# caskcsg/lightretriever

Hardware: AMD Instinct MI355X
Metric: docs embedded/sec (llama3.2-1b dims, seq_len=512, bf16) [+ queries/sec@top-100 over 1000000-doc index in `search`] (higher is better)
Workload: dtype bf16

## Files before the change

lightretriever_amd/csrc/lrx_search.hip:

```cpp
#include "lrx_common.h"
#include <float.h>
#include <stdlib.h>

typedef const __attribute__((address_space(1))) void* gptr_t;
typedef __attribute__((address_space(3))) void* lptr_t;

#define ROWS_F32 0
#define ROWS_F16T 1

#include "lrx_search_filter.h"

extern "C" int64_t lrx_flat_ip_score_ld(int64_t n_rows) { return lrx_cdiv(n_rows > 0 ? n_rows : 1, S_ROWS) * S_ROWS; }

#define SPLIT_MIN_QT 3
static size_t split_ws_bytes(int32_t dim) { return (size_t)(dim / 32) * 3 * 8 * 1024; }

struct FilterMode {
  int bmode = 0;
  int ss = 1;
  int unit = 1;
  int64_t nblocks = -1;
  const float* thr = nullptr;
  unsigned long long* cand = nullptr;
  unsigned int* cnt = nullptr;
  unsigned int cap = CAND_CAP_MIN;
  int* zero = nullptr;
  int nzero = 0;
  PreSplit presplit;
  bool planes_ready = false;
  bool group_max = false;
  const struct FusedArgs* fused = nullptr;
  bool range = false;
};
struct FusedArgs {
  int64_t ld_s;
  int nblk_s, nblk_ld_s, nsamp, nmain, ss, k;
  const float* bounds;
  float *thr, *eps;
  unsigned long long* cand;
  unsigned int* cnt;
  unsigned int cap;
  FusedCtl* ctl;
  int phases;
  int rs;
};

static int lrx_cu_count() {
  static const int n_cu = []() {
    int dev = 0;
    hipDeviceProp_t prop;
    return (hipGetDevice(&dev) == hipSuccess && hipGetDeviceProperties(&prop, dev) == hipSuccess && prop.multiProcessorCount > 0) ? prop.multiProcessorCount : 256;
  }();
  return n_cu;
}

static int filter_rows_per_wg(bool shadow) { return shadow ? 128 : 16 * SPF_RT * SPF_WV; }
template <int RS>
static int launch_filter_fused(const void* Xs, int64_t n_rows, int dim, const __bf16* qsplit, int nq, int qt, float* scores, float* gmax, const float* qf32,
                               const FusedArgs& fa, hipStream_t s);

static int launch_scores(const float* X, int64_t n_rows, int64_t ldx, int32_t dim, const float* q, int32_t n_queries, float* scores,
                         float* blkmax, __bf16* qsplit, void* stream, int planes = 3, const int* gate = nullptr, const void* Xs = nullptr,
                         int64_t ld = 0, const FilterMode& fm = FilterMode()) {
  LRX_CHECK_ARG(dim > 0 && dim % S_BK == 0, "flat_ip: dim=%d must be a multiple of %d", dim, S_BK);
  LRX_CHECK_ARG(ldx >= dim && ldx % 4 == 0, "flat_ip: ldx=%lld must be >= dim and a multiple of 4", (long long)ldx);
  if (n_rows <= 0 || n_queries <= 0) return LRX_OK;
  const int64_t ld_full = lrx_flat_ip_score_ld(n_rows);
  if (ld == 0) ld = ld_full;
  const int nblk_ld = (int)((ld / SP_ROWS + 3) & ~3);
  dim3 block(256);
  hipStream_t s = (hipStream_t)stream;
  const bool emit = fm.cand != nullptr;
  const bool shadow_pass = qsplit != nullptr && planes == 1 && Xs != nullptr;
  const int chunk = shadow_pass ? 256 : 128;
  LRX_CHECK_ARG(fm.bmode == 0 || (planes == 1 && qsplit != nullptr && n_queries <= chunk), "flat_ip: sampled filter launch outside the bounded search");
  for (int q0 = 0; q0 < n_queries; q0 += chunk) {
    int nq = n_queries - q0 < chunk ? n_queries - q0 : chunk;
    int qt = (nq + 15) / 16;
    const float* qp = q + (int64_t)q0 * dim;
    float* sp = scores ? scores + (int64_t)q0 * ld : nullptr;
    float* bp = blkmax ? blkmax + (int64_t)q0 * nblk_ld : nullptr;
    if (shadow_pass) {
      const int64_t nwg = fm.nblocks >= 0 ? fm.nblocks : ld_full / 128;
      if (nwg == 0) continue;
      if (fm.bmode != 2) {
        int threads = (dim / 64) * 2 * qt * 64;
        PreSplit ps = fm.presplit;
        ps.nb_xb = (threads + 255) / 256;
        hipLaunchKernelGGL(k_pack_queries_xb, dim3(ps.nb_xb + (ps.ngroups > 0 ? ps.blocks[0] + ps.blocks[1] : 0)), dim3(256), 0, s, qp, nq, dim, qt, qsplit,
                           fm.zero, fm.nzero, ps);
      }
      if (fm.fused != nullptr) {
        const int rc = fm.fused->rs == ROWS_F16T ? launch_filter_fused<ROWS_F16T>(Xs, n_rows, dim, qsplit, nq, qt, sp, bp, qp, *fm.fused, s)
                                                 : launch_filter_fused<ROWS_F32>(Xs, n_rows, dim, qsplit, nq, qt, sp, bp, qp, *fm.fused, s);
        if (rc != LRX_OK) return rc;
        continue;
      }
      constexpr int XPF = 4;
#ifndef XPF_S
#define XPF_S 4
#endif
      const int n_cu = lrx_cu_count();
      const bool persistent = emit && gate == nullptr && (dim / 64) % XPF == 0 && fm.bmode != 1 && nwg < (1ll << 31);
      const bool two_blocks = !emit && fm.bmode == 1 && nwg < (1ll << 31) && nwg > lrx_cu_count();
      const bool persistent_store = two_blocks && fm.group_max && gate == nullptr && sp != nullptr && bp != nullptr && qt <= 8 && (dim / 64) % XPF == 0 &&
                                    (nwg + 1) / 2 > 2 * (int64_t)n_cu;
#define LRX_XP(QQ, RT_)                                                                                                                     \
  {                                                                                                                                         \
    const int64_t groups = (nwg + RT_ - 1) / RT_;                                                                                           \
    if (fm.range)                                                                                                                           \
      hipLaunchKernelGGL((k_filter_xreg_emit<QQ, (QQ == 8 ? 2 : XPF), RT_, true>), dim3((unsigned)(groups < n_cu ? groups : n_cu)), dim3(576), 0, s, \
                         (const __bf16*)Xs, n_rows, dim, qsplit, nq, (int)nwg, fm.bmode, fm.ss, fm.unit, fm.thr, fm.cand, fm.cnt, fm.cap);     \
    else                                                                                                                                    \
    hipLaunchKernelGGL((k_filter_xreg_emit<QQ, (QQ == 8 ? 2 : XPF), RT_>), dim3((unsigned)(groups < n_cu ? groups : n_cu)), dim3(576), 0, s, (const __bf16*)Xs, n_rows, \
                       dim, qsplit, nq, (int)nwg, fm.bmode, fm.ss, fm.unit, fm.thr, fm.cand, fm.cnt, fm.cap);                              \
  }
#define LRX_XN(QQ, EM_)                                                                                                                     \
  hipLaunchKernelGGL((k_filter_xreg<QQ, (EM_ ? XPF : XPF_S), EM_>), dim3((unsigned)nwg), dim3(576), 0, s, (const __bf16*)Xs, n_rows, dim, qsplit, nq, sp, ld, bp, \
                     nblk_ld, gate, fm.bmode, fm.ss, fm.unit, fm.thr, fm.cand, fm.cnt, (int)nwg, fm.group_max ? 1 : 0, fm.cap);
#define LRX_XN2(QQ)                                                                              \
  hipLaunchKernelGGL((k_filter_xreg<QQ, XPF, false, 2>), dim3((unsigned)((nwg + 1) / 2)), dim3(576), 0, s, (const __bf16*)Xs, n_rows, dim, qsplit, nq, sp, ld, bp, \
                     nblk_ld, gate, fm.bmode, fm.ss, fm.unit, fm.thr, fm.cand, fm.cnt, (int)nwg, fm.group_max ? 1 : 0, fm.cap);
#define LRX_XS(QQ)                                                     \
// ... 236 lines not shown
extern "C" int32_t lrx_flat_ip_bounded_chunk_queries(int64_t n_rows, int32_t dim, int32_t n_queries, int32_t k, int32_t flags, int32_t has_shadow) {
  return chunk_queries(n_rows, dim, n_queries > 0 ? n_queries : 1, k, has_shadow && dim % 64 == 0, flags & 3);
}

static size_t chunk_plans_bytes(int64_t n_rows, int32_t dim, int32_t nq, int32_t k, int mode, bool shadow) {
  size_t need = 0;
  const int chunk = chunk_queries(n_rows, dim, nq, k, shadow, mode);
  const int sizes[2] = {nq < chunk ? nq : chunk, nq > chunk ? nq % chunk : 0};
  for (int i = 0; i < 2; ++i)
    if (sizes[i] > 0) {
      size_t t = plan_chunk(n_rows, dim, sizes[i], k, shadow, mode, 0).total;
      const size_t tf = plan_chunk(n_rows, dim, sizes[i], k, shadow, mode, 1).total;
      t = tf > t ? tf : t;
      need = t > need ? t : need;
    }
  return need;
}

extern "C" size_t lrx_flat_ip_bounded_workspace_bytes(int64_t n_rows, int32_t dim, int32_t n_queries, int32_t k, int32_t flags) {
  const int32_t nq = n_queries > 0 ? n_queries : 1;
  const size_t need = lrx_flat_ip_workspace_bytes(n_rows, dim, nq < 128 ? nq : 128, k);
  const size_t a = chunk_plans_bytes(n_rows, dim, nq, k, flags & 3, false), b = chunk_plans_bytes(n_rows, dim, nq, k, flags & 3, true);
  const size_t m = a > b ? a : b;
  return (m > need ? m : need) + 512;
}

extern "C" int lrx_flat_ip_search_bounded(const float* X, int64_t n_rows, int64_t ldx, int32_t dim, const void* X_shadow, const float* row_bounds,
                                          const float* q, int32_t n_queries, int32_t k, int64_t id_base, float* out_scores, int64_t* out_ids,
                                          void* workspace, size_t workspace_bytes, int32_t flags, void* stream) {
  return lrx_flat_ip_search_bounded_wire(X, n_rows, ldx, dim, X_shadow, row_bounds, q, n_queries, k, id_base, out_scores, out_ids, nullptr, nullptr,
                                         workspace, workspace_bytes, flags, stream);
}

template <int RS>
static int bounded_search(const float* X, int64_t n_rows, int64_t ldx, int32_t dim, const void* X_shadow, const float* row_bounds,
                          const float* q, int32_t n_queries, int32_t k, int64_t id_base, float* out_scores, int64_t* out_ids,
                          const int64_t* row_map, uint64_t* out_wire, void* workspace, size_t workspace_bytes, int32_t flags, void* stream) {
  const int mode = flags & 3;
  const bool shadow = X_shadow != nullptr && dim % 64 == 0;
  const int qt_max = ((n_queries < 128 ? n_queries : 128) + 15) / 16;
  if (RS == ROWS_F32 && ((qt_max < SPLIT_MIN_QT && !shadow) || n_rows <= REF_CAND || dim % 4 != 0)) {
    for (int q0 = 0; q0 < n_queries; q0 += 128) {
      const int nq = n_queries - q0 < 128 ? n_queries - q0 : 128;
      const int rc = lrx_flat_ip_search(X, n_rows, ldx, dim, row_bounds, q + (int64_t)q0 * dim, nq, k, id_base, out_scores + (int64_t)q0 * k,
                                        out_ids + (int64_t)q0 * k, workspace, workspace_bytes, stream);
      if (rc != LRX_OK) return rc;
    }
    return out_wire != nullptr ? lrx_pack_topk(out_scores, out_ids, row_map, id_base, (int64_t)n_queries * k, out_wire, stream) : LRX_OK;
  }
  hipStream_t s = (hipStream_t)stream;
  const int chunk = chunk_queries(n_rows, dim, n_queries, k, shadow, mode);
  const int use_fused = fused_pref_of(flags);
  for (int q0 = 0; q0 < n_queries; q0 += chunk) {
    const int nq = n_queries - q0 < chunk ? n_queries - q0 : chunk;
    const BoundedPlan p = plan_chunk(n_rows, dim, nq, k, shadow, mode, use_fused);
    LRX_CHECK_ARG(nq <= (shadow ? 256 : 128) || (p.gemm && p.emit), "flat_ip_search_bounded: a chunk of %d queries without the GEMM main pass", nq);
    if (p.total > workspace_bytes) {
      lrx_set_error("flat_ip_search_bounded: chunk of %d queries needs %zu B of workspace, %zu given", nq, p.total, workspace_bytes);
      return LRX_ERR_WORKSPACE;
    }
    const float* qc = q + (int64_t)q0 * dim;
    float* osc = out_scores + (int64_t)q0 * k;
    int64_t* oic = out_ids + (int64_t)q0 * k;
    char* ws = (char*)workspace;
    float* scores = (float*)ws;
    __bf16* qsplit = (__bf16*)(ws + p.off_qsplit);
    int* flg = (int*)(ws + p.off_ints);
    int* any_flag = flg + nq;
    unsigned int* cnt = (unsigned int*)(flg + ints_before_cnt(nq));
    int* part_cnt = (int*)(cnt + (size_t)nq * CNT_STRIDE);
    float* thr = (float*)(part_cnt + (size_t)nq * REF_SPLIT);
    float* eps = thr + nq;
    unsigned long long* parts = (unsigned long long*)(ws + p.off_parts);
    unsigned long long* cand = (unsigned long long*)(ws + p.off_cand);
    const size_t nclear = ints_before_cnt(nq) + (p.emit ? (size_t)nq * CNT_STRIDE : 0);
    const bool clear_in_pack = shadow && nclear < (1u << 30);
    if (!clear_in_pack) LRX_HIP(hipMemsetAsync(flg, 0, sizeof(int) * nclear, s));
    __bf16* qs3 = (__bf16*)(ws + p.off_qs3);
    const int64_t qs3_stride = (int64_t)(split_ws_bytes(dim) / sizeof(__bf16));
    auto presplit_of = [&](int j) {
      PreSplit ps;
      if (!shadow || RS == ROWS_F16T) return ps;
      const int n0 = j * 256, nj = nq - n0 < 256 ? nq - n0 : 256;
      ps.qs3 = qs3 + (int64_t)(2 * j) * qs3_stride;
      ps.stride = qs3_stride;
      for (int f0 = 0, g = 0; f0 < nj; f0 += 128, ++g) {
        const int nf = nj - f0 < 128 ? nj - f0 : 128, qtf = (nf + 15) / 16;
        ps.nf[g] = nf;
        ps.qt[g] = qtf;
        ps.blocks[g] = qtf >= SPLIT_MIN_QT ? ((dim / 32) * qtf * 64 + 255) / 256 : 0;
        ps.ngroups = g + 1;
      }
      if (ps.blocks[0] + ps.blocks[1] == 0) ps.ngroups = 0;
      return ps;
    };
    const PreSplit presplit = presplit_of(0);
    int rc;
    int nsplit = REF_SPLIT;
    if (p.emit) {
      float* blkmax = scores + p.ld_s * (int64_t)nq;
      FilterMode fs;
      fs.bmode = 1; fs.ss = p.ss; fs.unit = 1; fs.nblocks = p.nsamp_wg;
      fs.group_max = shadow;
      if (clear_in_pack) { fs.zero = flg; fs.nzero = (int)nclear; }
      fs.presplit = presplit;
      FusedArgs fa;
      if (p.fused && clear_in_pack) {
        fa.ld_s = p.ld_s; fa.nblk_s = (int)p.nblk_s; fa.nblk_ld_s = (int)p.nblk_ld_s; fa.nsamp = (int)p.nsamp_wg; fa.nmain = (int)p.nmain_wg; fa.ss = p.ss; fa.k = k;
        fa.bounds = row_bounds; fa.thr = thr; fa.eps = eps; fa.cand = cand; fa.cnt = cnt; fa.cap = p.cap;
        fa.ctl = (FusedCtl*)(flg + ints_before_cnt(nq) - 8);
        static const int fused_stamps = lrx_dev_knob("LRX_FUSED_PHASES", 0) & 128;
        fa.phases = 7 | fused_stamps;
        fa.rs = RS;
        fs.fused = &fa;
      }
      __bf16* q16 = (__bf16*)(ws + p.off_q16);
      if (p.gemm) {
        for (int j = 0, n0 = 0; n0 < nq; ++j, n0 += 256) {
          const int nj = nq - n0 < 256 ? nq - n0 : 256, qtj = (nj + 15) / 16;
          PreSplit ps = presplit_of(j);
          ps.nb_xb = ((dim / 64) * 2 * qtj * 64 + 255) / 256;
          hipLaunchKernelGGL(k_pack_queries_xb, dim3(ps.nb_xb + (ps.ngroups > 0 ? ps.blocks[0] + ps.blocks[1] : 0)), dim3(256), 0, s, qc + (int64_t)n0 * dim, nj, dim, qtj,
                             qsplit, j == 0 ? fs.zero : (int*)nullptr, j == 0 ? fs.nzero : 0, ps);
          LRX_LAUNCH_CHECK();
        }
        hipLaunchKernelGGL(k_round_queries, dim3((unsigned)lrx_cdiv((int64_t)nq * dim, 1024)), dim3(256), 0, s, qc, (int64_t)nq * dim, q16);
        LRX_LAUNCH_CHECK();
        rc = lrx_gemm_filter_sample_launch(X_shadow, q16, n_rows, nq, dim, p.ss, p.nsamp_wg, scores, blkmax, p.ld_s, (int)p.nblk_ld_s, s);
      } else {
        rc = launch_scores(X, n_rows, ldx, dim, qc, nq, scores, blkmax, qsplit, stream, 1, nullptr, shadow ? X_shadow : nullptr, p.ld_s, fs);
      }
      if (rc != LRX_OK) return rc;
      if (fs.fused == nullptr)
      hipLaunchKernelGGL(k_sample_threshold<RS>, dim3(nq), dim3(SEL_THREADS), 0, s, (const float*)scores, p.ld_s, p.nsamp_wg * p.rb, k, (const float*)blkmax,
                         (int)p.nblk_s, (int)p.nblk_ld_s, qc, dim, row_bounds, p.rb, p.ss, n_rows, thr, eps, cand, cnt, fs.group_max ? 16 : 128, p.cap);
      LRX_LAUNCH_CHECK();
      if (fs.fused != nullptr) {
        rc = LRX_OK;
      } else if (p.gemm) {
        rc = lrx_gemm_filter_emit_launch(X_shadow, q16, n_rows, nq, dim, p.ss, p.nmain_wg, thr, cand, cnt, p.cap, s);
      } else {
        FilterMode fm;
        fm.bmode = 2; fm.ss = p.ss; fm.nblocks = p.nmain_wg; fm.thr = thr; fm.cand = cand; fm.cnt = cnt; fm.cap = p.cap;
        rc = launch_scores(X, n_rows, ldx, dim, qc, nq, nullptr, nullptr, qsplit, stream, 1, nullptr, shadow ? X_shadow : nullptr, p.ld, fm);
      }
      if (rc != LRX_OK) return rc;
      nsplit = (int64_t)nq * REF_SPLIT <= lrx_cu_count() ? REF_SPLIT : ((int64_t)nq * 2 <= lrx_cu_count() ? 2 : 1);
      RowPairs rp = {nullptr, nullptr, nullptr, 0};
      {
        const int gshift = dim <= 512 ? 5 : (dim <= 1024 ? 4 : (dim <= 2048 ? 3 : 2));
        const int64_t ngroups = (n_rows + ((int64_t)1 << gshift) - 1) >> gshift;
        const size_t pair_bytes = align256((size_t)nq * REF_CAND * 8);
        const size_t need = 2 * pair_bytes + align256((size_t)(ngroups + 2) * 4) * 2 + 256;
        const bool fits = need <= p.off_qsplit && ((int64_t)1 << gshift) * dim <= ROWGRP_LDS_FLOATS && dim % 4 == 0 && ldx % 4 == 0 && ngroups < (1 << 30);
        const bool rule = dim >= 2048 && (int64_t)nq * k * 5 / 4 >= (5 * n_rows) / 2;
        if (fits && !(flags & 32) && (rule || (flags & 16))) {
          char* b = ws;
          rp.pairs = (unsigned long long*)b;
          unsigned long long* sorted = (unsigned long long*)(b + pair_bytes);
          rp.grp_cnt = (unsigned int*)(b + 2 * pair_bytes);
          unsigned int* grp_off = (unsigned int*)(b + 2 * pair_bytes + align256((size_t)(ngroups + 2) * 4));
          rp.total = grp_off + ngroups + 1;
          rp.grp_shift = gshift;
          LRX_HIP(hipMemsetAsync(rp.grp_cnt, 0, (size_t)((char*)(rp.total + 1) - (char*)rp.grp_cnt), s));
          hipLaunchKernelGGL(k_refine_band<RS>, dim3(nq, nsplit), dim3(1024), 0, s, X, n_rows, ldx, dim, qc, (const unsigned long long*)cand,
                             (const unsigned int*)cnt, (const float*)eps, k, parts, part_cnt, nsplit, p.cap, rp);
          LRX_LAUNCH_CHECK();
          hipLaunchKernelGGL(k_pairs_scan, dim3(1), dim3(1024), 0, s, (const unsigned int*)rp.grp_cnt, grp_off, (int)ngroups);
          LRX_LAUNCH_CHECK();
          hipLaunchKernelGGL(k_pairs_scatter, dim3((unsigned)(4 * lrx_cu_count())), dim3(256), 0, s, (const unsigned long long*)rp.pairs, (const unsigned int*)rp.total,
                             rp.grp_cnt, (const unsigned int*)grp_off, gshift, sorted);
          LRX_LAUNCH_CHECK();
          hipLaunchKernelGGL(k_rescore_row_groups<RS>, dim3((unsigned)ngroups), dim3(ROWGRP_THREADS), 0, s, X, n_rows, ldx, dim, qc, (const unsigned long long*)sorted,
                             (const unsigned int*)grp_off, gshift, parts);
          LRX_LAUNCH_CHECK();
        }
      }
      if (rp.pairs == nullptr) {
        hipLaunchKernelGGL(k_refine_band<RS>, dim3(nq, nsplit), dim3(1024), 0, s, X, n_rows, ldx, dim, qc, (const unsigned long long*)cand,
                           (const unsigned int*)cnt, (const float*)eps, k, parts, part_cnt, nsplit, p.cap, rp);
        LRX_LAUNCH_CHECK();
      }
    } else {
      float* blkmax = scores + p.ld * (int64_t)nq;
      FilterMode fa;
      if (clear_in_pack) { fa.zero = flg; fa.nzero = (int)nclear; }
      fa.presplit = presplit;
      rc = launch_scores(X, n_rows, ldx, dim, qc, nq, scores, blkmax, qsplit, stream, 1, nullptr, shadow ? X_shadow : nullptr, 0, fa);
      if (rc != LRX_OK) return rc;
      hipLaunchKernelGGL(k_topk_select, dim3(nq), dim3(SEL_THREADS), 0, s, (const float*)scores, p.ld, n_rows, k, id_base, (const float*)blkmax, (int)p.nblk,
                         (int)p.nblk_ld, osc, oic, (const int*)nullptr, (const int*)nullptr);
      LRX_LAUNCH_CHECK();
      hipLaunchKernelGGL(k_refine_topk<RS>, dim3(nq, REF_SPLIT), dim3(1024), 0, s, X, n_rows, ldx, dim, qc, (const float*)scores, p.ld, (const float*)blkmax,
                         (int)p.nblk, (int)p.nblk_ld, row_bounds, k, id_base, (const float*)osc, parts, part_cnt);
      LRX_LAUNCH_CHECK();
    }
    hipLaunchKernelGGL(k_refine_merge, dim3(nq), dim3(1024), 0, s, (const unsigned long long*)parts, (const int*)part_cnt, n_rows, k, id_base, osc, oic,
                       flg, any_flag, nsplit);
    LRX_LAUNCH_CHECK();
    for (int f0 = 0; f0 < nq; f0 += 128) {
      const int nf = nq - f0 < 128 ? nq - f0 : 128;
      float* blkmax = scores + p.ld * (int64_t)nf;
      FilterMode ff;
      const PreSplit psf = presplit_of(f0 / 256);
      ff.planes_ready = psf.ngroups > 0;
      const int* gate = any_flag + f0 / 128;
      if (RS == ROWS_F16T)
        rc = launch_scores(nullptr, n_rows, dim, dim, qc + (int64_t)f0 * dim, nf, scores, blkmax, qsplit, stream, 1, gate, X_shadow, 0, FilterMode());
      else
        rc = launch_scores(X, n_rows, ldx, dim, qc + (int64_t)f0 * dim, nf, scores, blkmax, ff.planes_ready ? qs3 + (f0 / 128) * qs3_stride : qsplit, stream, 3,
                           gate, nullptr, 0, ff);
      if (rc != LRX_OK) return rc;
      hipLaunchKernelGGL(k_topk_select_rescore<RS>, dim3(nf), dim3(SEL_THREADS), 0, s, (const float*)scores, p.ld, n_rows, k, id_base, (const float*)blkmax,
                         (int)p.nblk, (int)p.nblk_ld, X, ldx, dim, qc + (int64_t)f0 * dim, osc + (int64_t)f0 * k, oic + (int64_t)f0 * k,
                         gate, (const int*)(flg + f0), row_bounds,
                         out_wire != nullptr ? (unsigned long long*)out_wire + ((int64_t)q0 + f0) * k : (unsigned long long*)nullptr, row_map);
      LRX_LAUNCH_CHECK();
    }
  }
  return LRX_OK;
}

extern "C" int lrx_flat_ip_search_bounded_wire(const float* X, int64_t n_rows, int64_t ldx, int32_t dim, const void* X_shadow, const float* row_bounds,
                                               const float* q, int32_t n_queries, int32_t k, int64_t id_base, float* out_scores, int64_t* out_ids,
                                               const int64_t* row_map, uint64_t* out_wire, void* workspace, size_t workspace_bytes, int32_t flags,
                                               void* stream) {
  LRX_CHECK_ARG(row_bounds != nullptr, "flat_ip_search_bounded: null row_bounds (device pointer to {max |x_row|, max |x_row - fp16(x_row)|})");
  LRX_CHECK_ARG(k > 0 && k <= SEL_MAXK, "flat_ip_search: k=%d out of range (1..%d)", k, SEL_MAXK);
  LRX_CHECK_ARG(n_rows >= 0 && n_rows < (1ll << 32), "flat_ip_search: shard rows=%lld out of range", (long long)n_rows);
  LRX_CHECK_ARG((flags & ~63) == 0 && (flags & 12) != 12 && (flags & 48) != 48, "flat_ip_search_bounded: unknown flags 0x%x", flags);
  if (n_queries <= 0) return LRX_OK;
  if (workspace_bytes < lrx_flat_ip_bounded_workspace_bytes(n_rows, dim, n_queries, k, flags)) {
    lrx_set_error("flat_ip_search_bounded: workspace %zu B < required %zu B", workspace_bytes, lrx_flat_ip_bounded_workspace_bytes(n_rows, dim, n_queries, k, flags));
    return LRX_ERR_WORKSPACE;
  }
  return bounded_search<ROWS_F32>(X, n_rows, ldx, dim, X_shadow, row_bounds, q, n_queries, k, id_base, out_scores, out_ids, row_map, out_wire,
                                  workspace, workspace_bytes, flags, stream);
}
// ... 436 lines not shown
```

lightretriever_amd/csrc/lrx_search_filter.h:

```cpp
#pragma once

typedef __attribute__((ext_vector_type(8))) _Float16 f16x8;
__device__ __forceinline__ f32x4 mfma_f16(bf16x8 a, bf16x8 b, f32x4 c) {
  return __builtin_amdgcn_mfma_f32_16x16x32_f16(__builtin_bit_cast(f16x8, a), __builtin_bit_cast(f16x8, b), c, 0, 0, 0);
}
__device__ __forceinline__ _Float16 f2h_sat(float v) { return (_Float16)fminf(fmaxf(v, -65504.f), 65504.f); }
__device__ __forceinline__ __bf16 f2h_bits(float v) { return __builtin_bit_cast(__bf16, f2h_sat(v)); }

#define S_ROWS 256
#define S_BK 32
#define S_XTILE (S_ROWS * S_BK * 4)
#define SP_ROWS 128

template <int QT>
__global__ void __launch_bounds__(256, 1)
k_flat_ip_scores(const float* __restrict__ X, int64_t N, int64_t ldx, int D, const float* __restrict__ Q, int nq,
                 float* __restrict__ scores, int64_t ld, float* __restrict__ blkmax, int nblk, const int* __restrict__ gate) {
  constexpr int QTILE = QT * 16 * S_BK * 4;
  constexpr int STAGE = S_XTILE + QTILE;
  __shared__ __attribute__((aligned(1024))) char smem[2 * STAGE];
  if (gate != nullptr && *gate == 0) return;
  const int tid = threadIdx.x, lane = tid & 63, wave = tid >> 6;
  const int64_t n0 = (int64_t)blockIdx.x * S_ROWS;

// ... 100 lines not shown
  m = (__bf16)r1;
  float r2 = r1 - (float)m;
  l = (__bf16)r2;
}

__device__ __forceinline__ void split_queries_body(const float* __restrict__ Q, int nq, int D, int QT, int NP, __bf16* __restrict__ qs, int gid) {
  int lane = gid & 63, rest = gid >> 6;
  int qt = rest % QT, kt = rest / QT;
  if (kt >= D / 32) return;
  int fi = lane & 15, fq = lane >> 4;
  int row = qt * 16 + fi;
  bf16x8 h, m, l;
#pragma unroll
  for (int j = 0; j < 8; ++j) {
    int k = kt * 32 + (j < 4 ? 4 * fq + j : 16 + 4 * fq + (j - 4));
    float v = row < nq ? Q[(int64_t)row * D + k] : 0.f;
    __bf16 a, b, c;
    split3(v, a, b, c);
    h[j] = NP == 1 ? f2h_bits(v) : a; m[j] = b; l[j] = c;
  }
  int64_t base = (((int64_t)kt * NP) * QT + qt) * 64 + lane;
  bf16x8* out = (bf16x8*)qs;
  out[base] = h;
  if (NP == 3) {
    out[base + (int64_t)QT * 64] = m;
    out[base + 2 * (int64_t)QT * 64] = l;
  }
}
__global__ void k_split_queries(const float* __restrict__ Q, int nq, int D, int QT, int NP, __bf16* __restrict__ qs, const int* __restrict__ gate) {
  if (gate != nullptr && *gate == 0) return;
  split_queries_body(Q, nq, D, QT, NP, qs, blockIdx.x * blockDim.x + threadIdx.x);
}

struct PreSplit {
  __bf16* qs3 = nullptr;
  int64_t stride = 0;
  int ngroups = 0, nb_xb = 0;
  int nf[2] = {0, 0}, qt[2] = {0, 0}, blocks[2] = {0, 0};
};

__global__ void k_pack_queries_xb(const float* __restrict__ Q, int nq, int D, int QT, __bf16* __restrict__ qs, int* __restrict__ zero, int nzero,
                                  PreSplit ps) {
  if (ps.ngroups > 0 && (int)blockIdx.x >= ps.nb_xb) {
    int b = (int)blockIdx.x - ps.nb_xb, g = 0;
    if (b >= ps.blocks[0]) { b -= ps.blocks[0]; g = 1; }
    split_queries_body(Q + (int64_t)g * 128 * D, ps.nf[g], D, ps.qt[g], 3, ps.qs3 + g * ps.stride, b * blockDim.x + threadIdx.x);
    return;
  }
  const int nb = ps.ngroups > 0 ? ps.nb_xb : (int)gridDim.x;
  int gid = blockIdx.x * blockDim.x + threadIdx.x;
  for (int i = gid; i < nzero; i += nb * blockDim.x) zero[i] = 0;
  int lane = gid & 63, rest = gid >> 6;
  int qt = rest % QT, r2 = rest / QT;
  int ks = r2 & 1, sl = r2 >> 1;
  if (sl >= D / 64) return;
  int fi = lane & 15, fq = lane >> 4;
  int row = qt * 16 + fi;
  bf16x8 h;
#pragma unroll
  for (int j = 0; j < 8; ++j) h[j] = f2h_bits(row < nq ? Q[(int64_t)row * D + sl * 64 + ks * 32 + fq * 8 + j] : 0.f);
  ((bf16x8*)qs)[(((int64_t)sl * 2 + ks) * QT + qt) * 64 + lane] = h;
}

__global__ void k_round_queries(const float* __restrict__ Q, int64_t n, __bf16* __restrict__ q16) {
  const int64_t i = ((int64_t)blockIdx.x * blockDim.x + threadIdx.x) * 4;
  if (i >= n) return;
  const f32x4 v = *(const f32x4*)(Q + i);
  bf16x4 o;
#pragma unroll
  for (int e = 0; e < 4; ++e) o[e] = f2h_bits(v[e]);
  *(bf16x4*)(q16 + i) = o;
}

#ifndef SPF_RT
#define SPF_RT 2
#endif
#ifndef SPF_NST
#define SPF_NST 2
#endif
#ifndef SPF_WV
#define SPF_WV 8
#endif
template <int QT, int NP, int RT, int NST, int WV, bool EMIT = false>
__global__ void __launch_bounds__(64 * WV, ((NST * (16 * RT * WV * 128 + ((NP * QT + WV - 1) / WV) * WV * 1024) <= 81920) ? 2 : 1))
// ... 973 lines not shown
```

lightretriever_amd/csrc/lrx_search_refine.h:

```cpp
#pragma once

template <int RS>
__device__ __forceinline__ void refine_rescore(const float* __restrict__ X, int64_t ldx, int D, const float* qrow, const unsigned long long* s_cand,
                                               int nc, unsigned long long* __restrict__ mine) {
  const int lane = threadIdx.x & 63, wave = threadIdx.x >> 6;
  for (int c0 = wave * 2; c0 < nc; c0 += 32) {
    const int c = min(c0 + (lane >> 5), nc - 1);
    const int64_t n = (int64_t)s_cand[c];
    const float sc = row_dot<RS>(X, ldx, n, qrow, D, lane);
    if ((lane & 31) == 0 && c0 + (lane >> 5) < nc) mine[c] = sel_pack(f2key(sc), n);
  }
}

struct RowPairs {
  unsigned long long* pairs;
  unsigned int* total;
  unsigned int* grp_cnt;
  int grp_shift;
};
template <int RS>
__global__ void __launch_bounds__(1024)
k_refine_band(const float* __restrict__ X, int64_t N, int64_t ldx, int D, const float* __restrict__ q, const unsigned long long* __restrict__ cand,
              const unsigned int* __restrict__ cnt, const float* __restrict__ eps, int k, unsigned long long* __restrict__ parts,
              int* __restrict__ part_cnt, int nsplit, unsigned int cap, RowPairs rp) {
  __shared__ RadixShared rs;
  __shared__ unsigned long long s_cand[REF_CAND];
  __shared__ __attribute__((aligned(16))) float s_q[REF_QLDS];
  __shared__ unsigned int s_ncand;
  const int tid = threadIdx.x;
  const int qi = blockIdx.x, part = blockIdx.y;
  const unsigned int pcand = REF_CAND / nsplit;
  const float* qglob = q + (int64_t)qi * D;
  const float* qrow = D <= REF_QLDS ? s_q : qglob;
  if (D <= REF_QLDS)
    for (int i = tid; i < D; i += 1024) s_q[i] = qglob[i];
  if (tid == 0) s_ncand = 0;
  const unsigned int n = cnt[qi * CNT_STRIDE];
  bool overflow = n > cap || n < (unsigned int)k;
  __syncthreads();
  if (!overflow) {
    const unsigned long long* list = cand + (int64_t)qi * cap;
    const float kth = key2f(radix_select_kth_list(list, (int)n, (unsigned int)k, rs));
    const float thr = kth - 2.0f * eps[qi];
    for (int i = part + nsplit * tid; i < (int)n; i += nsplit * 1024) {
      const unsigned long long e = list[i];
      if (key2f((uint32_t)(e >> 32)) >= thr) {
        const int64_t row = sel_row(e);
        const unsigned int p = row < N ? atomicAdd(&s_ncand, 1u) : atomicAdd(&s_ncand, (unsigned int)REF_CAND + 1u);
        if (p < pcand) s_cand[p] = (unsigned long long)row;
      }
    }
    __syncthreads();
    overflow = s_ncand > pcand;
  }
  const int nc = overflow ? 0 : (int)s_ncand;
  if (rp.pairs != nullptr) {
    __shared__ unsigned int s_base;
    if (tid == 0) s_base = nc > 0 ? atomicAdd(rp.total, (unsigned int)nc) : 0u;
    __syncthreads();
    const unsigned int slot0 = (unsigned int)((qi * nsplit + part) * (int)pcand);
    for (int c = tid; c < nc; c += 1024) {
      const unsigned long long row = s_cand[c];
      rp.pairs[s_base + c] = (row << 32) | (unsigned long long)(slot0 + (unsigned int)c);
      atomicAdd(&rp.grp_cnt[row >> rp.grp_shift], 1u);
    }
  } else {
    refine_rescore<RS>(X, ldx, D, qrow, s_cand, nc, parts + ((int64_t)qi * nsplit + part) * pcand);
  }
  if (tid == 0) part_cnt[qi * nsplit + part] = overflow ? -1 : nc;
}

__global__ void __launch_bounds__(1024)
k_pairs_scan(const unsigned int* __restrict__ grp_cnt, unsigned int* __restrict__ grp_off, int ngroups) {
  __shared__ unsigned int s_w[16];
  const int tid = threadIdx.x, lane = tid & 63, wave = tid >> 6;
  const int per = (ngroups + 1 + 1023) / 1024;
  const int g0 = tid * per, g1 = min(g0 + per, ngroups + 1);
  unsigned int mine = 0;
  for (int g = g0; g < g1; ++g) mine += g < ngroups ? grp_cnt[g] : 0u;
  unsigned int x = mine;
#pragma unroll
  for (int o = 1; o < 64; o <<= 1) { const unsigned int y = __shfl_up(x, o, 64); if (lane >= o) x += y; }
  if (lane == 63) s_w[wave] = x;
  __syncthreads();
  unsigned int run = x - mine;
  for (int w = 0; w < wave; ++w) run += s_w[w];
  for (int g = g0; g < g1; ++g) {
    grp_off[g] = run;
// ... 99 lines not shown
      const unsigned int p = atomicAdd(&s_nblk, 1u);
      if (p < REF_PBLK) s_blk[p] = (unsigned int)b;
    }
  __syncthreads();
  const unsigned int nb = s_nblk;
  bool overflow = nb > REF_PBLK;
  if (!overflow) {
    const float* row = scores + (int64_t)qi * ld;
    const unsigned int total = nb * SP_ROWS;
    for (unsigned int idx0 = tid; idx0 < total; idx0 += 4 * 1024) {
      float v[4];
      int64_t n[4];
#pragma unroll
      for (int u = 0; u < 4; ++u) {
        const unsigned int idx = idx0 + u * 1024;
        n[u] = idx < total ? (int64_t)s_blk[idx >> 7] * SP_ROWS + (idx & (SP_ROWS - 1)) : N;
        v[u] = n[u] < N ? row[n[u]] : -FLT_MAX;
      }
#pragma unroll
      for (int u = 0; u < 4; ++u)
        if (n[u] < N && v[u] >= thr) {
          const unsigned int p = atomicAdd(&s_ncand, 1u);
          if (p < REF_PCAND) s_cand[p] = (unsigned long long)n[u];
        }
    }
    __syncthreads();
    overflow = s_ncand > REF_PCAND;
  }
  const int nc = overflow ? 0 : (int)s_ncand;
  refine_rescore<RS>(X, ldx, D, qrow, s_cand, nc, parts + ((int64_t)qi * REF_SPLIT + part) * REF_PCAND);
  if (tid == 0) part_cnt[qi * REF_SPLIT + part] = overflow ? -1 : nc;
}

__device__ unsigned int g_search_fallback_queries = 0;
extern "C" int64_t lrx_search_fallback_count(int32_t reset) {
  unsigned int v = 0;
  if (hipMemcpyFromSymbol(&v, HIP_SYMBOL(g_search_fallback_queries), sizeof(v)) != hipSuccess) return -1;
  if (reset && v) {
    const unsigned int z = 0;
    if (hipMemcpyToSymbol(HIP_SYMBOL(g_search_fallback_queries), &z, sizeof(z)) != hipSuccess) return -1;
  }
  return (int64_t)v;
}

__global__ void __launch_bounds__(1024)
k_refine_merge(const unsigned long long* __restrict__ parts, const int* __restrict__ part_cnt, int64_t N, int k, int64_t id_base,
               float* __restrict__ out_scores, int64_t* __restrict__ out_ids, int* __restrict__ qflags, int* __restrict__ any_flag, int nsplit) {
  __shared__ unsigned long long s_cand[REF_CAND];
  const int tid = threadIdx.x, qi = blockIdx.x;
  const int pcand = REF_CAND / nsplit;
  float* os = out_scores + (int64_t)qi * k;
  int64_t* oi = out_ids + (int64_t)qi * k;
  const int keff = (int)(N < (int64_t)k ? N : (int64_t)k);
  if (keff == 0) return;
  int cnt[REF_SPLIT], tot = 0;
  bool any_over = false;
#pragma unroll
  for (int p = 0; p < REF_SPLIT; ++p) {
    cnt[p] = p < nsplit ? part_cnt[qi * nsplit + p] : 0;
    any_over |= cnt[p] < 0;
    tot += cnt[p] < 0 ? 0 : cnt[p];
  }
  if (any_over || tot < keff) {
    if (tid == 0) { qflags[qi] = 1; atomicOr(any_flag + (qi >> 7), 1); atomicAdd(&g_search_fallback_queries, 1u); }
    return;
  }
  int base = 0;
#pragma unroll
  for (int p = 0; p < REF_SPLIT; ++p) {
    const unsigned long long* src = parts + ((int64_t)qi * nsplit + p) * pcand;
    for (int i = tid; i < cnt[p]; i += blockDim.x) s_cand[base + i] = src[i];
    base += cnt[p];
  }
  __syncthreads();
  if (tot <= (int)blockDim.x) {
    if (tid < tot) {
      const unsigned long long me = s_cand[tid];
      int r = 0;
      int j = 0;
      for (; j + 4 <= tot; j += 4)
        r += (s_cand[j] > me ? 1 : 0) + (s_cand[j + 1] > me ? 1 : 0) + (s_cand[j + 2] > me ? 1 : 0) + (s_cand[j + 3] > me ? 1 : 0);
      for (; j < tot; ++j) r += s_cand[j] > me ? 1 : 0;
      if (r < keff) {
        os[r] = key2f((uint32_t)(me >> 32));
        oi[r] = id_base + sel_row(me);
      }
    }
    return;
  }
  int P = 1;
  while (P < tot) P <<= 1;
  for (int i = tot + tid; i < P; i += blockDim.x) s_cand[i] = 0ull;
  if (P == 2 * (int)blockDim.x) bitonic_sort_desc_regs<2>(s_cand, P);
  else if (P == 4 * (int)blockDim.x) bitonic_sort_desc_regs<4>(s_cand, P);
  else bitonic_sort_desc(s_cand, P);
  for (int i = tid; i < keff; i += blockDim.x) {
    const unsigned long long c = s_cand[i];
    os[i] = key2f((uint32_t)(c >> 32));
    oi[i] = id_base + sel_row(c);
  }
}
```

Measured before the change: 1365.

## Defer query 3-plane split to fallback queries and add fused refine-merge path

Removes the eager pre-split of queries into three bf16 planes that ran inside the pack kernel for every batch. The split now runs only for queries flagged for exhaustive fallback, from within the refine/merge kernels via a shared helper. Adds an optional single-block refine kernel variant (gated by an env knob, off by default) that rescores candidates and writes the top-k directly, skipping the separate merge launch. This trades unconditional split work for per-query work on the fallback path, which adds some load to the merge kernel when fallbacks occur.

```diff
diff --git a/lightretriever_amd/csrc/lrx_search.hip b/lightretriever_amd/csrc/lrx_search.hip
--- a/lightretriever_amd/csrc/lrx_search.hip
+++ b/lightretriever_amd/csrc/lrx_search.hip
@@ -26,7 +26,6 @@
   unsigned int cap = CAND_CAP_MIN;
   int* zero = nullptr;
   int nzero = 0;
-  PreSplit presplit;
   bool planes_ready = false;
   bool group_max = false;
   const struct FusedArgs* fused = nullptr;
@@ -85,10 +84,7 @@
       if (nwg == 0) continue;
       if (fm.bmode != 2) {
         int threads = (dim / 64) * 2 * qt * 64;
-        PreSplit ps = fm.presplit;
-        ps.nb_xb = (threads + 255) / 256;
-        hipLaunchKernelGGL(k_pack_queries_xb, dim3(ps.nb_xb + (ps.ngroups > 0 ? ps.blocks[0] + ps.blocks[1] : 0)), dim3(256), 0, s, qp, nq, dim, qt, qsplit,
-                           fm.zero, fm.nzero, ps);
+        hipLaunchKernelGGL(k_pack_queries_xb, dim3((threads + 255) / 256), dim3(256), 0, s, qp, nq, dim, qt, qsplit, fm.zero, fm.nzero);
       }
       if (fm.fused != nullptr) {
         const int rc = fm.fused->rs == ROWS_F16T ? launch_filter_fused<ROWS_F16T>(Xs, n_rows, dim, qsplit, nq, qt, sp, bp, qp, *fm.fused, s)
@@ -391,6 +387,12 @@
                                          workspace, workspace_bytes, flags, stream);
 }
 
+static bool refine_one_rule(int64_t n_rows, int32_t dim, int32_t nq, int32_t k) {
+  static const int force = lrx_dev_knob("LRX_REFINE_ONE", 0);
+  (void)n_rows; (void)dim; (void)k;
+  return force == 1 && nq <= lrx_cu_count();
+}
+
 template <int RS>
 static int bounded_search(const float* X, int64_t n_rows, int64_t ldx, int32_t dim, const void* X_shadow, const float* row_bounds,
                           const float* q, int32_t n_queries, int32_t k, int64_t id_base, float* out_scores, int64_t* out_ids,
@@ -437,32 +439,16 @@
     if (!clear_in_pack) LRX_HIP(hipMemsetAsync(flg, 0, sizeof(int) * nclear, s));
     __bf16* qs3 = (__bf16*)(ws + p.off_qs3);
     const int64_t qs3_stride = (int64_t)(split_ws_bytes(dim) / sizeof(__bf16));
-    auto presplit_of = [&](int j) {
-      PreSplit ps;
-      if (!shadow || RS == ROWS_F16T) return ps;
-      const int n0 = j * 256, nj = nq - n0 < 256 ? nq - n0 : 256;
-      ps.qs3 = qs3 + (int64_t)(2 * j) * qs3_stride;
-      ps.stride = qs3_stride;
-      for (int f0 = 0, g = 0; f0 < nj; f0 += 128, ++g) {
-        const int nf = nj - f0 < 128 ? nj - f0 : 128, qtf = (nf + 15) / 16;
-        ps.nf[g] = nf;
-        ps.qt[g] = qtf;
-        ps.blocks[g] = qtf >= SPLIT_MIN_QT ? ((dim / 32) * qtf * 64 + 255) / 256 : 0;
-        ps.ngroups = g + 1;
-      }
-      if (ps.blocks[0] + ps.blocks[1] == 0) ps.ngroups = 0;
-      return ps;
-    };
-    const PreSplit presplit = presplit_of(0);
+    const FallbackPlanes planes = {RS == ROWS_F32 && dim % S_BK == 0 ? qs3 : (__bf16*)nullptr, qs3_stride, qc, nq, dim};
     int rc;
     int nsplit = REF_SPLIT;
+    bool merged = false;
     if (p.emit) {
       float* blkmax = scores + p.ld_s * (int64_t)nq;
       FilterMode fs;
       fs.bmode = 1; fs.ss = p.ss; fs.unit = 1; fs.nblocks = p.nsamp_wg;
       fs.group_max = shadow;
       if (clear_in_pack) { fs.zero = flg; fs.nzero = (int)nclear; }
-      fs.presplit = presplit;
       FusedArgs fa;
       if (p.fused && clear_in_pack) {
         fa.ld_s = p.ld_s; fa.nblk_s = (int)p.nblk_s; fa.nblk_ld_s = (int)p.nblk_ld_s; fa.nsamp = (int)p.nsamp_wg; fa.nmain = (int)p.nmain_wg; fa.ss = p.ss; fa.k = k;
@@ -475,12 +461,8 @@
       }
       __bf16* q16 = (__bf16*)(ws + p.off_q16);
       if (p.gemm) {
-        for (int j = 0, n0 = 0; n0 < nq; ++j, n0 += 256) {
-          const int nj = nq - n0 < 256 ? nq - n0 : 256, qtj = (nj + 15) / 16;
-          PreSplit ps = presplit_of(j);
-          ps.nb_xb = ((dim / 64) * 2 * qtj * 64 + 255) / 256;
-          hipLaunchKernelGGL(k_pack_queries_xb, dim3(ps.nb_xb + (ps.ngroups > 0 ? ps.blocks[0] + ps.blocks[1] : 0)), dim3(256), 0, s, qc + (int64_t)n0 * dim, nj, dim, qtj,
-                             qsplit, j == 0 ? fs.zero : (int*)nullptr, j == 0 ? fs.nzero : 0, ps);
+        if (clear_in_pack) {
+          hipLaunchKernelGGL(k_pack_queries_xb, dim3((unsigned)lrx_cdiv((int64_t)fs.nzero, 1024)), dim3(256), 0, s, qc, 0, 0, 1, qsplit, fs.zero, fs.nzero);
           LRX_LAUNCH_CHECK();
         }
         hipLaunchKernelGGL(k_round_queries, dim3((unsigned)lrx_cdiv((int64_t)nq * dim, 1024)), dim3(256), 0, s, qc, (int64_t)nq * dim, q16);
@@ -523,7 +505,7 @@
           rp.grp_shift = gshift;
           LRX_HIP(hipMemsetAsync(rp.grp_cnt, 0, (size_t)((char*)(rp.total + 1) - (char*)rp.grp_cnt), s));
           hipLaunchKernelGGL(k_refine_band<RS>, dim3(nq, nsplit), dim3(1024), 0, s, X, n_rows, ldx, dim, qc, (const unsigned long long*)cand,
-                             (const unsigned int*)cnt, (const float*)eps, k, parts, part_cnt, nsplit, p.cap, rp);
+                             (const unsigned int*)cnt, (const float*)eps, k, parts, part_cnt, nsplit, p.cap, rp, MergeOut());
           LRX_LAUNCH_CHECK();
           hipLaunchKernelGGL(k_pairs_scan, dim3(1), dim3(1024), 0, s, (const unsigned int*)rp.grp_cnt, grp_off, (int)ngroups);
           LRX_LAUNCH_CHECK();
@@ -535,16 +517,21 @@
           LRX_LAUNCH_CHECK();
         }
       }
-      if (rp.pairs == nullptr) {
+      if (rp.pairs == nullptr && refine_one_rule(n_rows, dim, nq, k)) {
+        const MergeOut mo = {id_base, osc, oic, flg, any_flag, planes};
+        hipLaunchKernelGGL((k_refine_band<RS, true>), dim3(nq, 1), dim3(1024), 0, s, X, n_rows, ldx, dim, qc, (const unsigned long long*)cand,
+                           (const unsigned int*)cnt, (const float*)eps, k, parts, part_cnt, 1, p.cap, rp, mo);
+        LRX_LAUNCH_CHECK();
+        merged = true;
+      } else if (rp.pairs == nullptr) {
         hipLaunchKernelGGL(k_refine_band<RS>, dim3(nq, nsplit), dim3(1024), 0, s, X, n_rows, ldx, dim, qc, (const unsigned long long*)cand,
-                           (const unsigned int*)cnt, (const float*)eps, k, parts, part_cnt, nsplit, p.cap, rp);
+                           (const unsigned int*)cnt, (const float*)eps, k, parts, part_cnt, nsplit, p.cap, rp, MergeOut());
         LRX_LAUNCH_CHECK();
       }
     } else {
       float* blkmax = scores + p.ld * (int64_t)nq;
       FilterMode fa;
       if (clear_in_pack) { fa.zero = flg; fa.nzero = (int)nclear; }
-      fa.presplit = presplit;
       rc = launch_scores(X, n_rows, ldx, dim, qc, nq, scores, blkmax, qsplit, stream, 1, nullptr, shadow ? X_shadow : nullptr, 0, fa);
       if (rc != LRX_OK) return rc;
       hipLaunchKernelGGL(k_topk_select, dim3(nq), dim3(SEL_THREADS), 0, s, (const float*)scores, p.ld, n_rows, k, id_base, (const float*)blkmax, (int)p.nblk,
@@ -554,15 +541,16 @@
                          (int)p.nblk, (int)p.nblk_ld, row_bounds, k, id_base, (const float*)osc, parts, part_cnt);
       LRX_LAUNCH_CHECK();
     }
-    hipLaunchKernelGGL(k_refine_merge, dim3(nq), dim3(1024), 0, s, (const unsigned long long*)parts, (const int*)part_cnt, n_rows, k, id_base, osc, oic,
-                       flg, any_flag, nsplit);
-    LRX_LAUNCH_CHECK();
+    if (!merged) {
+      hipLaunchKernelGGL(k_refine_merge, dim3(nq), dim3(1024), 0, s, (const unsigned long long*)parts, (const int*)part_cnt, n_rows, k, id_base, osc, oic,
+                         flg, any_flag, nsplit, planes);
+      LRX_LAUNCH_CHECK();
+    }
     for (int f0 = 0; f0 < nq; f0 += 128) {
       const int nf = nq - f0 < 128 ? nq - f0 : 128;
       float* blkmax = scores + p.ld * (int64_t)nf;
       FilterMode ff;
-      const PreSplit psf = presplit_of(f0 / 256);
-      ff.planes_ready = psf.ngroups > 0;
+      ff.planes_ready = planes.qs3 != nullptr && (nf + 15) / 16 >= SPLIT_MIN_QT;
       const int* gate = any_flag + f0 / 128;
       if (RS == ROWS_F16T)
         rc = launch_scores(nullptr, n_rows, dim, dim, qc + (int64_t)f0 * dim, nf, scores, blkmax, qsplit, stream, 1, gate, X_shadow, 0, FilterMode());
diff --git a/lightretriever_amd/csrc/lrx_search_filter.h b/lightretriever_amd/csrc/lrx_search_filter.h
--- a/lightretriever_amd/csrc/lrx_search_filter.h
+++ b/lightretriever_amd/csrc/lrx_search_filter.h
@@ -156,24 +156,29 @@
   split_queries_body(Q, nq, D, QT, NP, qs, blockIdx.x * blockDim.x + threadIdx.x);
 }
 
-struct PreSplit {
-  __bf16* qs3 = nullptr;
-  int64_t stride = 0;
-  int ngroups = 0, nb_xb = 0;
-  int nf[2] = {0, 0}, qt[2] = {0, 0}, blocks[2] = {0, 0};
-};
-
-__global__ void k_pack_queries_xb(const float* __restrict__ Q, int nq, int D, int QT, __bf16* __restrict__ qs, int* __restrict__ zero, int nzero,
-                                  PreSplit ps) {
-  if (ps.ngroups > 0 && (int)blockIdx.x >= ps.nb_xb) {
-    int b = (int)blockIdx.x - ps.nb_xb, g = 0;
-    if (b >= ps.blocks[0]) { b -= ps.blocks[0]; g = 1; }
-    split_queries_body(Q + (int64_t)g * 128 * D, ps.nf[g], D, ps.qt[g], 3, ps.qs3 + g * ps.stride, b * blockDim.x + threadIdx.x);
-    return;
-  }
-  const int nb = ps.ngroups > 0 ? ps.nb_xb : (int)gridDim.x;
+__device__ __forceinline__ void split_query_row(const float* __restrict__ qrow, int D, int QT, int ql, __bf16* __restrict__ qs) {
+  const int qt = ql >> 4, fi = ql & 15;
+  bf16x8* out = (bf16x8*)qs;
+  for (int t = threadIdx.x; t < (D / 32) * 4; t += blockDim.x) {
+    const int kt = t >> 2, fq = t & 3;
+    bf16x8 h, m, l;
+#pragma unroll
+    for (int j = 0; j < 8; ++j) {
+      const int k = kt * 32 + (j < 4 ? 4 * fq + j : 16 + 4 * fq + (j - 4));
+      __bf16 a, b, c;
+      split3(qrow[k], a, b, c);
+      h[j] = a; m[j] = b; l[j] = c;
+    }
+    const int64_t base = (((int64_t)kt * 3) * QT + qt) * 64 + fq * 16 + fi;
+    out[base] = h;
+    out[base + (int64_t)QT * 64] = m;
+    out[base + 2 * (int64_t)QT * 64] = l;
+  }
+}
+
+__global__ void k_pack_queries_xb(const float* __restrict__ Q, int nq, int D, int QT, __bf16* __restrict__ qs, int* __restrict__ zero, int nzero) {
   int gid = blockIdx.x * blockDim.x + threadIdx.x;
-  for (int i = gid; i < nzero; i += nb * blockDim.x) zero[i] = 0;
+  for (int i = gid; i < nzero; i += gridDim.x * blockDim.x) zero[i] = 0;
   int lane = gid & 63, rest = gid >> 6;
   int qt = rest % QT, r2 = rest / QT;
   int ks = r2 & 1, sl = r2 >> 1;
diff --git a/lightretriever_amd/csrc/lrx_search_refine.h b/lightretriever_amd/csrc/lrx_search_refine.h
--- a/lightretriever_amd/csrc/lrx_search_refine.h
+++ b/lightretriever_amd/csrc/lrx_search_refine.h
@@ -2,7 +2,7 @@
 
 template <int RS>
 __device__ __forceinline__ void refine_rescore(const float* __restrict__ X, int64_t ldx, int D, const float* qrow, const unsigned long long* s_cand,
-                                               int nc, unsigned long long* __restrict__ mine) {
+                                               int nc, unsigned long long* mine) {
   const int lane = threadIdx.x & 63, wave = threadIdx.x >> 6;
   for (int c0 = wave * 2; c0 < nc; c0 += 32) {
     const int c = min(c0 + (lane >> 5), nc - 1);
@@ -12,17 +12,79 @@
   }
 }
 
+__device__ unsigned int g_search_fallback_queries = 0;
+extern "C" int64_t lrx_search_fallback_count(int32_t reset) {
+  unsigned int v = 0;
+  if (hipMemcpyFromSymbol(&v, HIP_SYMBOL(g_search_fallback_queries), sizeof(v)) != hipSuccess) return -1;
+  if (reset && v) {
+    const unsigned int z = 0;
+    if (hipMemcpyToSymbol(HIP_SYMBOL(g_search_fallback_queries), &z, sizeof(z)) != hipSuccess) return -1;
+  }
+  return (int64_t)v;
+}
+
+struct FallbackPlanes {
+  __bf16* qs3;
+  int64_t stride;
+  const float* q;
+  int nq, D;
+};
+__device__ __forceinline__ void refine_flag_query(int qi, int* __restrict__ qflags, int* __restrict__ any_flag, const FallbackPlanes& fp) {
+  if (threadIdx.x == 0) { qflags[qi] = 1; atomicOr(any_flag + (qi >> 7), 1); atomicAdd(&g_search_fallback_queries, 1u); }
+  if (fp.qs3 != nullptr) {
+    const int g = qi >> 7, nf = min(128, fp.nq - (g << 7)), qtf = (nf + 15) >> 4;
+    if (qtf >= SPLIT_MIN_QT) split_query_row(fp.q + (int64_t)qi * fp.D, fp.D, qtf, qi & 127, fp.qs3 + g * fp.stride);
+  }
+}
+__device__ __forceinline__ void refine_write_topk(unsigned long long* s_cand, int tot, int keff, int64_t id_base, float* __restrict__ os,
+                                                  int64_t* __restrict__ oi) {
+  const int tid = threadIdx.x;
+  if (tot <= (int)blockDim.x) {
+    if (tid < tot) {
+      const unsigned long long me = s_cand[tid];
+      int r = 0;
+      int j = 0;
+      for (; j + 4 <= tot; j += 4)
+        r += (s_cand[j] > me ? 1 : 0) + (s_cand[j + 1] > me ? 1 : 0) + (s_cand[j + 2] > me ? 1 : 0) + (s_cand[j + 3] > me ? 1 : 0);
+      for (; j < tot; ++j) r += s_cand[j] > me ? 1 : 0;
+      if (r < keff) {
+        os[r] = key2f((uint32_t)(me >> 32));
+        oi[r] = id_base + sel_row(me);
+      }
+    }
+    return;
+  }
+  int P = 1;
+  while (P < tot) P <<= 1;
+  for (int i = tot + tid; i < P; i += blockDim.x) s_cand[i] = 0ull;
+  if (P == 2 * (int)blockDim.x) bitonic_sort_desc_regs<2>(s_cand, P);
+  else if (P == 4 * (int)blockDim.x) bitonic_sort_desc_regs<4>(s_cand, P);
+  else bitonic_sort_desc(s_cand, P);
+  for (int i = tid; i < keff; i += blockDim.x) {
+    const unsigned long long c = s_cand[i];
+    os[i] = key2f((uint32_t)(c >> 32));
+    oi[i] = id_base + sel_row(c);
+  }
+}
+
 struct RowPairs {
   unsigned long long* pairs;
   unsigned int* total;
   unsigned int* grp_cnt;
   int grp_shift;
 };
-template <int RS>
+struct MergeOut {
+  int64_t id_base;
+  float* out_scores;
+  int64_t* out_ids;
+  int *qflags, *any_flag;
+  FallbackPlanes fp;
+};
+template <int RS, bool MERGE = false>
 __global__ void __launch_bounds__(1024)
 k_refine_band(const float* __restrict__ X, int64_t N, int64_t ldx, int D, const float* __restrict__ q, const unsigned long long* __restrict__ cand,
               const unsigned int* __restrict__ cnt, const float* __restrict__ eps, int k, unsigned long long* __restrict__ parts,
-              int* __restrict__ part_cnt, int nsplit, unsigned int cap, RowPairs rp) {
+              int* __restrict__ part_cnt, int nsplit, unsigned int cap, RowPairs rp, MergeOut mo) {
   __shared__ RadixShared rs;
   __shared__ unsigned long long s_cand[REF_CAND];
   __shared__ __attribute__((aligned(16))) float s_q[REF_QLDS];
@@ -54,6 +116,17 @@
     overflow = s_ncand > pcand;
   }
   const int nc = overflow ? 0 : (int)s_ncand;
+  if constexpr (MERGE) {
+    const int keff = (int)(N < (int64_t)k ? N : (int64_t)k);
+    if (overflow || nc < keff) {
+      refine_flag_query(qi, mo.qflags, mo.any_flag, mo.fp);
+      return;
+    }
+    refine_rescore<RS>(X, ldx, D, qrow, s_cand, nc, s_cand);
+    __syncthreads();
+    refine_write_topk(s_cand, nc, keff, mo.id_base, mo.out_scores + (int64_t)qi * k, mo.out_ids + (int64_t)qi * k);
+    return;
+  }
   if (rp.pairs != nullptr) {
     __shared__ unsigned int s_base;
     if (tid == 0) s_base = nc > 0 ? atomicAdd(rp.total, (unsigned int)nc) : 0u;
@@ -219,25 +292,13 @@
   if (tid == 0) part_cnt[qi * REF_SPLIT + part] = overflow ? -1 : nc;
 }
 
-__device__ unsigned int g_search_fallback_queries = 0;
-extern "C" int64_t lrx_search_fallback_count(int32_t reset) {
-  unsigned int v = 0;
-  if (hipMemcpyFromSymbol(&v, HIP_SYMBOL(g_search_fallback_queries), sizeof(v)) != hipSuccess) return -1;
-  if (reset && v) {
-    const unsigned int z = 0;
-    if (hipMemcpyToSymbol(HIP_SYMBOL(g_search_fallback_queries), &z, sizeof(z)) != hipSuccess) return -1;
-  }
-  return (int64_t)v;
-}
-
 __global__ void __launch_bounds__(1024)
 k_refine_merge(const unsigned long long* __restrict__ parts, const int* __restrict__ part_cnt, int64_t N, int k, int64_t id_base,
-               float* __restrict__ out_scores, int64_t* __restrict__ out_ids, int* __restrict__ qflags, int* __restrict__ any_flag, int nsplit) {
+               float* __restrict__ out_scores, int64_t* __restrict__ out_ids, int* __restrict__ qflags, int* __restrict__ any_flag, int nsplit,
+               FallbackPlanes fp) {
   __shared__ unsigned long long s_cand[REF_CAND];
   const int tid = threadIdx.x, qi = blockIdx.x;
   const int pcand = REF_CAND / nsplit;
-  float* os = out_scores + (int64_t)qi * k;
-  int64_t* oi = out_ids + (int64_t)qi * k;
   const int keff = (int)(N < (int64_t)k ? N : (int64_t)k);
   if (keff == 0) return;
   int cnt[REF_SPLIT], tot = 0;
@@ -249,7 +310,7 @@
     tot += cnt[p] < 0 ? 0 : cnt[p];
   }
   if (any_over || tot < keff) {
-    if (tid == 0) { qflags[qi] = 1; atomicOr(any_flag + (qi >> 7), 1); atomicAdd(&g_search_fallback_queries, 1u); }
+    refine_flag_query(qi, qflags, any_flag, fp);
     return;
   }
   int base = 0;
@@ -260,30 +321,5 @@
     base += cnt[p];
   }
   __syncthreads();
-  if (tot <= (int)blockDim.x) {
-    if (tid < tot) {
-      const unsigned long long me = s_cand[tid];
-      int r = 0;
-      int j = 0;
-      for (; j + 4 <= tot; j += 4)
-        r += (s_cand[j] > me ? 1 : 0) + (s_cand[j + 1] > me ? 1 : 0) + (s_cand[j + 2] > me ? 1 : 0) + (s_cand[j + 3] > me ? 1 : 0);
-      for (; j < tot; ++j) r += s_cand[j] > me ? 1 : 0;
-      if (r < keff) {
-        os[r] = key2f((uint32_t)(me >> 32));
-        oi[r] = id_base + sel_row(me);
-      }
-    }
-    return;
-  }
-  int P = 1;
-  while (P < tot) P <<= 1;
-  for (int i = tot + tid; i < P; i += blockDim.x) s_cand[i] = 0ull;
-  if (P == 2 * (int)blockDim.x) bitonic_sort_desc_regs<2>(s_cand, P);
-  else if (P == 4 * (int)blockDim.x) bitonic_sort_desc_regs<4>(s_cand, P);
-  else bitonic_sort_desc(s_cand, P);
-  for (int i = tid; i < keff; i += blockDim.x) {
-    const unsigned long long c = s_cand[i];
-    os[i] = key2f((uint32_t)(c >> 32));
-    oi[i] = id_base + sel_row(c);
-  }
-}
+  refine_write_topk(s_cand, tot, keff, id_base, out_scores + (int64_t)qi * k, out_ids + (int64_t)qi * k);
+}
```

Result: no change. 1365, median of 3 (-0.0%).
